# Litianyu141/Gen-FVGN-steady

Measured on AMD Instinct MI355X. Metric: training iters/sec, 50k-cell cylinder mesh (fwd + loss + bwd + Adam, batch resident in HBM), higher is better.
Workload: dtype f32

## Files before the change

### gen-fvgn-steady_amd/csrc/dw.hip

```cpp
#include <stdlib.h>
#include "gfv_common.h"
#include "gfv_prof.h"
#include "gfv_split.h"
#include "../../include/gfv.h"

__device__ int g_gfv_status_flags = 0;

extern "C" int gfv_status_flags(int32_t* flags_out) {
  int v = 0;
  if (hipMemcpyFromSymbol(&v, HIP_SYMBOL(g_gfv_status_flags), sizeof(int)) != hipSuccess) return GFV_ERR_LAUNCH;
  if (v) {
    const int zero = 0;
    if (hipMemcpyToSymbol(HIP_SYMBOL(g_gfv_status_flags), &zero, sizeof(int)) != hipSuccess) return GFV_ERR_LAUNCH;
  }
  if (flags_out) *flags_out = v;
  return GFV_OK;
}

int* gfv_internal_status_ptr() {
  static int* p = nullptr;
  if (!p) {
    void* q = nullptr;
    if (hipGetSymbolAddress(&q, HIP_SYMBOL(g_gfv_status_flags)) == hipSuccess) p = static_cast<int*>(q);
  }
// ... 186 lines not shown
    __syncthreads();
    buf ^= 1;
  }

  float* ws = A.ws + (size_t)slab * A.ws_stride + T.out_off;
#pragma unroll
  for (int i = 0; i < 4; ++i)
#pragma unroll
    for (int j = 0; j < 4; ++j)
#pragma unroll
      for (int reg = 0; reg < 4; ++reg) {
        const int n = 64 * wn + 16 * i + 4 * q + reg;
        const int k = 64 * wk + 16 * j + nl;
        if (FULL || (n < T.n_out && k < T.width)) ws[(size_t)n * T.ld_out + k] = acc[i][j][reg];
      }

  if (T.db_off >= 0) {
    float* red = lds;
    *reinterpret_cast<float4*>(&red[rg * LDT + col]) = dbacc;
    __syncthreads();
    if (tid < T.n_out) {
      float s = 0.f;
#pragma unroll
      for (int r = 0; r < 8; ++r) s += red[r * LDT + tid];
      A.ws[(size_t)slab * A.ws_stride + T.db_off + tid] = s;
    }
  }
}


constexpr int HBLK = 1024;
constexpr int HOP = 16 * HBLK;
constexpr int HBUF = 2 * HOP;
#ifdef GFV_DW_SINGLEBUF
constexpr int HSTAGE = HBUF;
#else
constexpr int HSTAGE = 2 * HBUF;
#endif

template <bool FULL, bool BF>
__device__ __forceinline__ void dw_body_h(const DwLaunch& A, const gfv_dw_tile_t& Tin, unsigned char* lds) {
  gfv_dw_tile_t T = Tin;
  const bool colscale = (T.a_op & GFV_DW_COLSCALE) != 0;
  T.a_op &= 7;
  const int tid = threadIdx.x, wave = tid >> 6, lane = tid & 63, nl = lane & 15, q = lane >> 4;
  const int wn = wave >> 1, wk = wave & 1;
  const int slab = blockIdx.x;
  const int kpad = FULL ? 128 : ((T.width + 15) & ~15);
  const int npad = FULL ? 128 : ((T.n_out + 15) & ~15);
  const bool gvec = FULL || (((T.ldg & 3) == 0) && ((T.n_out & 3) == 0));
  const bool avec = FULL || (((T.ld & 3) == 0) && ((T.width & 3) == 0));
  const int c4 = tid & 31, r4 = tid >> 5;
  const int col = 4 * c4;
  float4 gam = make_float4(1.f, 1.f, 1.f, 1.f), bet = make_float4(0.f, 0.f, 0.f, 0.f);
  if (T.a_op == 2) {
    gam = *reinterpret_cast<const float4*>(T.a_gamma + col);
    bet = *reinterpret_cast<const float4*>(T.a_beta + col);
  }
  const int m_beg = slab * A.rows_per_slab;
  const int m_end = min(m_beg + A.rows_per_slab, A.M);

  float* wred = reinterpret_cast<float*>(lds);
  float sg;
  if (T.gscale) {
    float smin = 8.5070592e37f;
    for (int q = (m_beg >> 4) + tid; q < ((m_end + 15) >> 4); q += 256) smin = fminf(smin, T.gscale[q]);
    smin = gfv_wave_min(smin);
    if (lane == 0) wred[wave] = smin;
    __syncthreads();
    sg = fminf(fminf(wred[0], wred[1]), fminf(wred[2], wred[3]));
    __syncthreads();
  } else {
    float gm = 0.f;
    for (int m = m_beg + r4; m < m_end; m += 64) {
      float4 v[8];
#pragma unroll
      for (int u = 0; u < 8; ++u) v[u] = ld4(T.G, (size_t)min(m + 8 * u, m_end - 1), T.ldg, col, FULL ? 128 : T.n_out, gvec);
#pragma unroll
      for (int u = 0; u < 8; ++u)
        gm = fmaxf(fmaxf(gm, fmaxf(fabsf(v[u].x), fabsf(v[u].y))), fmaxf(fabsf(v[u].z), fabsf(v[u].w)));
    }
    gm = gfv_wave_max(gm);
    if (lane == 0) wred[wave] = gm;
    __syncthreads();
    sg = gfv_pow2_scale(fmaxf(fmaxf(wred[0], wred[1]), fmaxf(wred[2], wred[3])));
    __syncthreads();
  }

  float4 sa = make_float4(1.f, 1.f, 1.f, 1.f);
  if (colscale && m_beg < m_end) {
    float4 cm = make_float4(0.f, 0.f, 0.f, 0.f);
    for (int m = m_beg + r4; m < m_end; m += 64) {
      float4 v[8], b[8];
#pragma unroll
      for (int u = 0; u < 8; ++u) {
        const int mm = min(m + 8 * u, m_end - 1);
        const size_t row = T.idx ? (size_t)T.idx[mm] : (size_t)mm;
        v[u] = ld4(T.A, row, T.ld, col, FULL ? 128 : T.width, avec);
        b[u] = T.in_add ? ld4(T.in_add, row, T.ld, col, FULL ? 128 : T.width, avec) : make_float4(0.f, 0.f, 0.f, 0.f);
      }
#pragma unroll
      for (int u = 0; u < 8; ++u) {
        cm.x = fmaxf(cm.x, fabsf(v[u].x + b[u].x)); cm.y = fmaxf(cm.y, fabsf(v[u].y + b[u].y));
        cm.z = fmaxf(cm.z, fabsf(v[u].z + b[u].z)); cm.w = fmaxf(cm.w, fabsf(v[u].w + b[u].w));
      }
    }
    *reinterpret_cast<float4*>(&wred[r4 * 128 + col]) = cm;
    __syncthreads();
#pragma unroll
    for (int r = 0; r < 8; ++r) {
      const float4 o = *reinterpret_cast<const float4*>(&wred[r * 128 + col]);
      cm.x = fmaxf(cm.x, o.x); cm.y = fmaxf(cm.y, o.y); cm.z = fmaxf(cm.z, o.z); cm.w = fmaxf(cm.w, o.w);
    }
    sa = make_float4(gfv_pow2_scale(cm.x), gfv_pow2_scale(cm.y), gfv_pow2_scale(cm.z), gfv_pow2_scale(cm.w));
    __syncthreads();
  }
  float* inv_sa = reinterpret_cast<float*>(lds + HSTAGE);
  if (r4 == 0) *reinterpret_cast<float4*>(&inv_sa[col]) = make_float4(1.0f / sa.x, 1.0f / sa.y, 1.0f / sa.z, 1.0f / sa.w);
  float amax = 0.f;

  floatx4 acc[4][4];
#pragma unroll
  for (int i = 0; i < 4; ++i)
#pragma unroll
    for (int j = 0; j < 4; ++j) acc[i][j] = floatx4{0.f, 0.f, 0.f, 0.f};
  float4 dbacc = make_float4(0.f, 0.f, 0.f, 0.f);
  float4 greg[4], areg[4], breg[4];
  int nidx[4];
  auto load_idx = [&](int m0) {
#pragma unroll
    for (int p = 0; p < 4; ++p) {
      const int m = min(m0 + 4 * r4 + p, m_end - 1);
      nidx[p] = T.idx ? T.idx[m] : m;
    }
  };
  auto load_sub = [&](int m0) {
    size_t srow[4];
#pragma unroll
    for (int p = 0; p < 4; ++p) srow[p] = (size_t)nidx[p];
#pragma unroll
    for (int p = 0; p < 4; ++p) {
      const int m = min(m0 + 4 * r4 + p, m_end - 1);
      greg[p] = ld4(T.G, (size_t)m, T.ldg, col, FULL ? 128 : T.n_out, gvec);
    }
#pragma unroll
    for (int p = 0; p < 4; ++p) {
      areg[p] = ld4(T.A, srow[p], T.ld, col, FULL ? 128 : T.width, avec);
      if (T.in_add) breg[p] = ld4(T.in_add, srow[p], T.ld, col, FULL ? 128 : T.width, avec);
    }
    load_idx(m0 + SUB);
  };
  const int slot = ((r4 >> 1) * 16) * 16 + 8 * (r4 & 1);
  auto put4 = [&](unsigned char* op, int c, float v0, float v1, float v2, float v3) {
    unsigned h0, h1, l0, l1;
    gfv_split_pair_t<BF>(v0, v1, h0, l0);
    gfv_split_pair_t<BF>(v2, v3, h1, l1);
    unsigned char* b = op + ((c >> 4) * 2) * HBLK + ((c & 15) ^ ((c >> 4) & 3)) * 16 + slot;
    *reinterpret_cast<uint2*>(b) = make_uint2(h0, h1);
    *reinterpret_cast<uint2*>(b + HBLK) = make_uint2(l0, l1);
  };
  auto store_sub = [&](int buf, int m0) {
    unsigned char* Gs = lds + buf * HBUF;
    unsigned char* As = Gs + HOP;
    const float4 zero = make_float4(0.f, 0.f, 0.f, 0.f);
    float4 g[4], a[4];
#pragma unroll
    for (int p = 0; p < 4; ++p) {
      const bool live = (m0 + 4 * r4 + p) < m_end;
      g[p] = greg[p];
      a[p] = areg[p];
      if (T.in_add) { a[p].x += breg[p].x; a[p].y += breg[p].y; a[p].z += breg[p].z; a[p].w += breg[p].w; }
      if (T.a_op == 1) {
        a[p] = make_float4(gfv_gelu(a[p].x), gfv_gelu(a[p].y), gfv_gelu(a[p].z), gfv_gelu(a[p].w));
      } else if (T.a_op == 2) {
        const float mean = gfv_half_sum((a[p].x + a[p].y) + (a[p].z + a[p].w)) * A.ln_inv_n;
        const float dx = a[p].x - mean, dy = a[p].y - mean, dz = a[p].z - mean, dw = a[p].w - mean;
        const float var = (gfv_half_sum((dx * dx + dy * dy) + (dz * dz + dw * dw)) - A.ln_npad * (mean * mean)) * A.ln_inv_n;
        const float rstd = rsqrtf(var + 1e-5f);
        a[p] = make_float4(dx * rstd * gam.x + bet.x, dy * rstd * gam.y + bet.y, dz * rstd * gam.z + bet.z,
                           dw * rstd * gam.w + bet.w);
      }
      if (!live) { g[p] = zero; a[p] = zero; }
      dbacc.x += g[p].x; dbacc.y += g[p].y; dbacc.z += g[p].z; dbacc.w += g[p].w;
      a[p].x *= sa.x; a[p].y *= sa.y; a[p].z *= sa.z; a[p].w *= sa.w;
      amax = fmaxf(fmaxf(amax, fmaxf(fabsf(a[p].x), fabsf(a[p].y))), fmaxf(fabsf(a[p].z), fabsf(a[p].w)));
    }
    put4(Gs, col + 0, g[0].x * sg, g[1].x * sg, g[2].x * sg, g[3].x * sg);
    put4(Gs, col + 1, g[0].y * sg, g[1].y * sg, g[2].y * sg, g[3].y * sg);
    put4(Gs, col + 2, g[0].z * sg, g[1].z * sg, g[2].z * sg, g[3].z * sg);
    put4(Gs, col + 3, g[0].w * sg, g[1].w * sg, g[2].w * sg, g[3].w * sg);
    put4(As, col + 0, a[0].x, a[1].x, a[2].x, a[3].x);
    put4(As, col + 1, a[0].y, a[1].y, a[2].y, a[3].y);
    put4(As, col + 2, a[0].z, a[1].z, a[2].z, a[3].z);
    put4(As, col + 3, a[0].w, a[1].w, a[2].w, a[3].w);
  };

  int buf = 0;
  if (m_beg < m_end) {
    load_idx(m_beg);
    load_sub(m_beg);
    store_sub(0, m_beg);
  }
  __syncthreads();
  for (int m0 = m_beg; m0 < m_end; m0 += SUB) {
    const bool more = m0 + SUB < m_end;
    if (more) load_sub(m0 + SUB);
#ifdef GFV_DW_SINGLEBUF
    const unsigned char* Gs = lds;
#else
    const unsigned char* Gs = lds + buf * HBUF;
#endif
    const unsigned char* As = Gs + HOP;
    gfv_f16x8 gh[4], gl[4], ah[4], al[4];
#pragma unroll
    for (int i = 0; i < 4; ++i) {
      gh[i] = *reinterpret_cast<const gfv_f16x8*>(Gs + ((4 * wn + i) * 2 + 0) * HBLK + (lane ^ i) * 16);
      gl[i] = *reinterpret_cast<const gfv_f16x8*>(Gs + ((4 * wn + i) * 2 + 1) * HBLK + (lane ^ i) * 16);
      ah[i] = *reinterpret_cast<const gfv_f16x8*>(As + ((4 * wk + i) * 2 + 0) * HBLK + (lane ^ i) * 16);
      al[i] = *reinterpret_cast<const gfv_f16x8*>(As + ((4 * wk + i) * 2 + 1) * HBLK + (lane ^ i) * 16);
    }
    if constexpr (BF) {
#pragma unroll
      for (int i = 0; i < 4; ++i)
#pragma unroll
        for (int j = 0; j < 4; ++j)
          if (FULL || (64 * wn + 16 * i < npad && 64 * wk + 16 * j < kpad)) acc[i][j] = gfv_mma_hh<true>(gh[i], ah[j], acc[i][j]);
    } else {
#pragma unroll
      for (int term = 0; term < 3; ++term)
        if (term == 2 || !A.lowp)
#pragma unroll
          for (int i = 0; i < 4; ++i)
#pragma unroll
            for (int j = 0; j < 4; ++j)
              if (FULL || (64 * wn + 16 * i < npad && 64 * wk + 16 * j < kpad))
                acc[i][j] = __builtin_amdgcn_mfma_f32_16x16x32_f16(term == 0 ? gl[i] : gh[i], term == 1 ? al[j] : ah[j],
                                                                   acc[i][j], 0, 0, 0);
    }
#ifdef GFV_DW_SINGLEBUF
    __syncthreads();
    if (more) store_sub(0, m0 + SUB);
    __syncthreads();
#else
    if (more) store_sub(buf ^ 1, m0 + SUB);
    __syncthreads();
    buf ^= 1;
#endif
  }

  if (!(amax <= 65504.f)) atomicOr(&g_gfv_status_flags, GFV_FLAG_DW_RANGE);
  const float inv = 1.0f / sg;
  float* ws = A.ws + (size_t)slab * A.ws_stride + T.out_off;
#pragma unroll
  for (int j = 0; j < 4; ++j) {
    const int k = 64 * wk + 16 * j + nl;
    const float inva = inv_sa[k];
#pragma unroll
    for (int i = 0; i < 4; ++i)
#pragma unroll
      for (int reg = 0; reg < 4; ++reg) {
        const int n = 64 * wn + 16 * i + 4 * q + reg;
        if (FULL || (n < T.n_out && k < T.width)) ws[(size_t)n * T.ld_out + k] = (acc[i][j][reg] * inv) * inva;
      }
  }

  if (T.db_off >= 0) {
    float* red = reinterpret_cast<float*>(lds);
    *reinterpret_cast<float4*>(&red[r4 * LDT + col]) = dbacc;
    __syncthreads();
    if (tid < T.n_out) {
      float s = 0.f;
#pragma unroll
      for (int r = 0; r < 8; ++r) s += red[r * LDT + tid];
      A.ws[(size_t)slab * A.ws_stride + T.db_off + tid] = s;
    }
  }
}

__global__ __launch_bounds__(256, 2) void dw_multi_kernel(const DwLaunch A) {
  __shared__ __attribute__((aligned(16))) float lds[4 * SUB * LDT];
// ... 212 lines not shown
```

### gen-fvgn-steady_amd/csrc/lin1.hip

```cpp
#include <atomic>
#include <cstdlib>

#include "../../include/gfv.h"
#include "gfv_common.h"
#include "gfv_split.h"

int* gfv_internal_status_ptr();
extern "C" int gfv_hidden_size(void);

namespace {

__device__ __forceinline__ float l1_max3_abs(float m, float a, float b) {
  float r;
  asm("v_max3_f32 %0, %1, |%2|, |%3|" : "=v"(r) : "v"(m), "v"(a), "v"(b));
  return r;
}
__device__ __forceinline__ float l1_row_max4(float v) {
  float a, b;
  gfv_lane_xor16(v, a, b);
  v = fmaxf(a, b);
  gfv_lane_xor32(v, a, b);
  return fmaxf(a, b);
}

// ... 327 lines not shown
  }
  __syncthreads();
  float* red = reinterpret_cast<float*>(lds_raw);
#pragma unroll
  for (int nt = 0; nt < 8; ++nt)
#pragma unroll
    for (int r = 0; r < 4; ++r) {
      const float dg = gfv_row16_sum(dgam[nt][r]), db = gfv_row16_sum(dbet[nt][r]);
      if (li == 0) {
        red[(wave * 2 + 0) * 128 + 16 * nt + 4 * g + r] = dg;
        red[(wave * 2 + 1) * 128 + 16 * nt + 4 * g + r] = db;
      }
    }
  __syncthreads();
  {
    const int half = tid >> 8, j = tid & 255;
    const int tile = 2 * blockIdx.x + half;
    if (tile < B.n_tiles && B.ln_partial) {
      const int w0 = 4 * half, which = j >> 7, c = j & 127;
      const float s = (red[((w0 + 0) * 2 + which) * 128 + c] + red[((w0 + 1) * 2 + which) * 128 + c]) +
                      (red[((w0 + 2) * 2 + which) * 128 + c] + red[((w0 + 3) * 2 + which) * 128 + c]);
      B.ln_partial[(size_t)tile * 256 + j] = s;
    }
  }
  (void)status;
}

struct Lin1CsrArgs {
  const float* src[2];
  int src_ld[2];
  const int* rowptr[2];
  const int* col[2];
  float* save[2];
  const void* img;
  const float* wmax;
  float* out;
  int out_ld;
  int M;
};
template <int LOWP>
__global__ __launch_bounds__(512, 2) void lin1_csr_kernel(const Lin1CsrArgs A, int* status) {
  constexpr int KS = 8;
  extern __shared__ __attribute__((aligned(16))) char lds_raw[];
  gfv_uint4* img = reinterpret_cast<gfv_uint4*>(lds_raw);
  const int tid = threadIdx.x, wave = tid >> 6, lane = tid & 63, li = lane & 15, g = lane >> 4;
  {
    const gfv_uint4* src = reinterpret_cast<const gfv_uint4*>(A.img);
    gfv_uint4 t[16];
#pragma unroll
    for (int u = 0; u < 16; ++u) t[u] = src[(size_t)u * 512 + tid];
#pragma unroll
    for (int u = 0; u < 16; ++u) img[u * 512 + tid] = t[u];
  }
  const int nwg = gridDim.x;
  const int wg = (nwg & 7) == 0 ? (int)(blockIdx.x & 7) * (nwg >> 3) + (int)(blockIdx.x >> 3) : (int)blockIdx.x;
  const int m = wg * 128 + 16 * wave + li;
  const bool live = m < A.M;
  const int mc = live ? m : A.M - 1;
  float v[KS][8];
#pragma unroll
  for (int T = 0; T < KS; ++T)
#pragma unroll
    for (int e = 0; e < 8; ++e) v[T][e] = 0.f;
  int kk[2], ee[2], cn0[2], cn1[2];
#pragma unroll
  for (int s = 0; s < 2; ++s) {
// ... 18 lines not shown
      const float* p0 = A.src[s] + (size_t)c0 * (size_t)A.src_ld[s] + 4 * g;
      const float* p1 = A.src[s] + (size_t)c1 * (size_t)A.src_ld[s] + 4 * g;
      if (one[s]) {
#pragma unroll
        for (int t = 0; t < 8; ++t) a0[s][t] = *reinterpret_cast<const float4*>(p0 + 16 * t);
      }
      if (two[s]) {
#pragma unroll
        for (int t = 0; t < 8; ++t) a1[s][t] = *reinterpret_cast<const float4*>(p1 + 16 * t);
      }
    }
#pragma unroll
    for (int s = 0; s < 2; ++s) {
#pragma unroll
      for (int t = 0; t < 8; ++t) {
        float* d = &v[4 * s + (t >> 1)][4 * (t & 1)];
        if (one[s]) { d[0] += a0[s][t].x; d[1] += a0[s][t].y; d[2] += a0[s][t].z; d[3] += a0[s][t].w; }
        if (two[s]) { d[0] += a1[s][t].x; d[1] += a1[s][t].y; d[2] += a1[s][t].z; d[3] += a1[s][t].w; }
      }
      kk[s] = min(kk[s] + 2, ee[s]);
    }
  }
#pragma unroll
  for (int s = 0; s < 2; ++s) {
    if (A.save[s] && live) {
#pragma unroll
      for (int T = 0; T < 4; ++T) {
        float* sp = A.save[s] + (size_t)m * 128 + 32 * T + 4 * g;
        *reinterpret_cast<float4*>(sp) = make_float4(v[4 * s + T][0], v[4 * s + T][1], v[4 * s + T][2], v[4 * s + T][3]);
        *reinterpret_cast<float4*>(sp + 16) = make_float4(v[4 * s + T][4], v[4 * s + T][5], v[4 * s + T][6], v[4 * s + T][7]);
      }
    }
  }
  float m0 = 0.f, m1 = 0.f;
#pragma unroll
  for (int T = 0; T < KS; ++T) {
    m0 = l1_max3_abs(m0, v[T][0], v[T][1]);
    m1 = l1_max3_abs(m1, v[T][2], v[T][3]);
    m0 = l1_max3_abs(m0, v[T][4], v[T][5]);
    m1 = l1_max3_abs(m1, v[T][6], v[T][7]);
  }
  const float sx = gfv_pow2_scale(l1_row_max4(fmaxf(m0, m1)));
  gfv_f16x8 xh[KS], xl[KS];
#pragma unroll
  for (int T = 0; T < KS; ++T) {
    float e[8];
#pragma unroll
    for (int i = 0; i < 8; ++i) e[i] = v[T][i] * sx;
    gfv_uint4 hi, lo;
    gfv_split8_t<LOWP == 2>(e, hi, lo);
    xh[T] = __builtin_bit_cast(gfv_f16x8, hi);
    xl[T] = __builtin_bit_cast(gfv_f16x8, lo);
  }
  const float inv = 1.0f / sx, invw = 1.0f / gfv_pow2_scale(*A.wmax);
  __syncthreads();
#pragma unroll 2
  for (int nt = 0; nt < 8; ++nt) {
    floatx4 acc = {0.f, 0.f, 0.f, 0.f};
#pragma unroll
    for (int T = 0; T < KS; ++T) {
      const gfv_uint4* f = img + (T * 8 + nt) * 128 + lane;
      const gfv_f16x8 wh = __builtin_bit_cast(gfv_f16x8, f[0]);
      if (!LOWP) {
        const gfv_f16x8 wl = __builtin_bit_cast(gfv_f16x8, f[64]);
        acc = __builtin_amdgcn_mfma_f32_16x16x32_f16(wl, xh[T], acc, 0, 0, 0);
        acc = __builtin_amdgcn_mfma_f32_16x16x32_f16(wh, xl[T], acc, 0, 0, 0);
      }
      acc = gfv_mma_hh<LOWP == 2>(wh, xh[T], acc);
    }
    if (live)
      *reinterpret_cast<float4*>(A.out + (size_t)m * A.out_ld + 16 * nt + 4 * g) =
          make_float4((acc[0] * inv) * invw, (acc[1] * inv) * invw, (acc[2] * inv) * invw, (acc[3] * inv) * invw);
  }
  (void)status;
}
// ... 7 lines not shown
static int l1_cus() {
  static int n = 0;
  if (!n) {
    int dev = 0;
    hipDeviceProp_t pr;
    if (hipGetDevice(&dev) == hipSuccess && hipGetDeviceProperties(&pr, dev) == hipSuccess) n = pr.multiProcessorCount;
    if (n <= 0) n = 256;
  }
  return n;
}
static inline bool l1_dyn_lds(const void* fn, int bytes, std::atomic<unsigned long long>& done) {
  int dev = 0;
  if (hipGetDevice(&dev) != hipSuccess) return false;
  const unsigned long long bit = 1ull << (dev & 63);
  if (done.load(std::memory_order_relaxed) & bit) return true;
  if (hipFuncSetAttribute(fn, hipFuncAttributeMaxDynamicSharedMemorySize, bytes) != hipSuccess) return false;
  done.fetch_or(bit);
  return true;
}
}

int gfv_internal_lin1s_try(const gfv_rowtile_args_t* a, int lowp, hipStream_t stream, int dry);
int gfv_internal_lin1_try(const gfv_rowtile_args_t* a, int lowp, hipStream_t stream, int dry) {
  static const int on = l1_env("GFV_LIN1", 1);
  if (on && gfv_internal_lin1s_try(a, lowp, stream, dry)) return 1;
  static const int min_m = l1_env("GFV_LIN1_MIN_M", 1024);
  if (!on || a->nlayers != 1 || a->M < min_m || (a->flags & (GFV_CHAIN_ROW_OWNER | GFV_CHAIN_COLUMN_OWNER))) return 0;
  const gfv_layer_t& L = a->layer[0];
  if (a->nseg == 2 && a->seg[0].csr_rowptr && a->seg[1].csr_rowptr) {
    static const int csr_on = l1_env("GFV_LIN1_CSR", 1);
    if (!csr_on || !L.Wh || !a->wmax || L.op != GFV_OP_NONE || L.save || L.aux || L.bias || L.bias2 || a->in_op != GFV_IN_NONE ||
        a->fin_op != GFV_FIN_PLAIN || L.K != 256 || L.N != 128)
      return 0;
    if (a->in_add || a->in_save || a->gscale || a->fin_presave || a->fin_stats || a->in_stats || a->dw_partial || a->gadd || a->padd ||
        a->in_aux || a->out_nores || a->ln_partial || a->res[0] || a->res[1] || a->res[2])
      return 0;
    if (!a->out[0] || a->out[1] || a->out[2] || (a->out_ld[0] & 3) || !al16(a->out[0])) return 0;
    Lin1CsrArgs B{};
    for (int i = 0; i < 2; ++i) {
      const gfv_seg_t& sg = a->seg[i];
      if (sg.width != 128 || !sg.idx || sg.csr_scale || (sg.ld & 3) || !al16(sg.ptr) || (sg.save && !al16(sg.save))) return 0;
      B.src[i] = sg.ptr; B.src_ld[i] = sg.ld; B.rowptr[i] = sg.csr_rowptr; B.col[i] = sg.idx; B.save[i] = sg.save;
    }
    B.img = L.Wh;
    B.wmax = a->wmax;
    B.out = a->out[0];
    B.out_ld = a->out_ld[0];
    B.M = a->M;
    if (dry) return 1;
    int* st = gfv_internal_status_ptr();
    const dim3 grid((a->M + 127) / 128), blk(512);
#define L1_CSR(LP)                                                                                               \
  do {                                                                                                           \
    static std::atomic<unsigned long long> done{0};                                                              \
    if (!l1_dyn_lds(reinterpret_cast<const void*>(&lin1_csr_kernel<LP>), 131072, done)) return 0;                \
    GFV_LAUNCH((lin1_csr_kernel<LP>), grid, blk, 131072, stream, B, st);                                 \
  } while (0)
    if (lowp == 2) L1_CSR(2);
    else if (lowp) L1_CSR(1);
    else L1_CSR(0);
#undef L1_CSR
    return 1;
  }
  if (a->fin_op == GFV_FIN_LNBWD) {
    static const int lnb_on = l1_env("GFV_LIN1_LNBWD", 1);
    if (!lnb_on || !L.Wh || !a->wmax || L.op != GFV_OP_NONE || L.save || L.aux || L.bias || L.bias2 || a->in_op != GFV_IN_NONE) return 0;
    if (a->nseg != 2 || L.K != 256 || L.N != 128 || a->in_add || a->in_save || a->gscale || a->fin_presave || a->fin_stats || a->in_stats ||
        a->dw_partial || a->gadd || a->padd || a->in_aux || a->out_nores || !a->fin_aux || !a->fin_gamma || !a->ln_partial)
      return 0;
    for (int i = 0; i < 2; ++i) {
      const gfv_seg_t& sg = a->seg[i];
      if (sg.width != 128 || sg.idx || sg.csr_rowptr || sg.csr_scale || sg.save || (sg.ld & 3) || !al16(sg.ptr)) return 0;
    }
    if (!a->out[0] || a->out[1] || a->out[2] || (a->out_ld[0] & 3) || !al16(a->out[0]) || a->res[1] || a->res[2]) return 0;
    if (a->res[0] && ((a->res_ld[0] & 3) || !al16(a->res[0]))) return 0;
// ... 116 lines not shown
```

### gen-fvgn-steady_amd/csrc/lin1s.hip

```cpp
#include <atomic>
#include <cstdlib>

#include "tchain_kernel.h"
#include "gfv_limits.h"

int* gfv_internal_status_ptr();
extern "C" int gfv_hidden_size(void);

namespace {

__device__ __forceinline__ void l1s_barrier() { asm volatile("s_waitcnt lgkmcnt(0)\n\ts_barrier" ::: "memory"); }

struct Lin1sArgs {
  const float* seg[2];
  int seg_ld[2];
  const int* rowptr[2];
  const int* col[2];
  float* save[2];
  const float* in_add;
  float* in_save;
  const void* img;
  const float* wmax;
  const float* bias[2];
  const float* res[2];
  int res_ld[2];
  float* out[2];
  int out_ld[2];
  int M;
  const float* gamma;
  const float* beta;
  float ln_inv_n, ln_npad;
  const float* aux;
  float* gscale;
  float* ln_partial;
};

template <int KS, int TG>
struct L1sLds {
  static constexpr int FRAG = 0;
  static constexpr int SINV = TG * KS * 2048;
  static constexpr int STAT = SINV + TG * 64;
  static constexpr int PART = STAT + TG * 128;
  static constexpr int TOTAL = PART + TG * 16 * 4 * 8;
};

template <int KS, int NP, int IN_OP, int EPI, bool CSR, int LOWP, int TG>
__global__ __launch_bounds__(256, 2) void lin1s_kernel(const Lin1sArgs A, int* status) {
  constexpr int NSEG = KS / 4;
  using LY = L1sLds<KS, TG>;
  constexpr bool BF = LOWP == 2;
  __shared__ __attribute__((aligned(16))) char lds[LY::TOTAL];
  float* sinv = reinterpret_cast<float*>(lds + LY::SINV);
  float* stat = reinterpret_cast<float*>(lds + LY::STAT);
  float* part = reinterpret_cast<float*>(lds + LY::PART);
  const int w = __builtin_amdgcn_readfirstlane(threadIdx.x >> 6);
  const int lane = threadIdx.x & 63, j = lane & 15, g = lane >> 4;
  const int tile = CSR ? gfv_xcd_tile(blockIdx.x, gridDim.x) : (int)blockIdx.x;
  const int row0 = tile * (16 * TG);
  if (row0 >= A.M) return;
  const int ngt = min(TG, (A.M - row0 + 15) >> 4);
  const int c0 = 32 * w + 4 * g;
  const float invw = 1.0f / gfv_pow2_scale(*A.wmax);

  gfv_f16x8 wh[2][KS], wl[2][KS];
  auto load_w = [&](int p) {
    const gfv_f16x8* im = reinterpret_cast<const gfv_f16x8*>(A.img) + (size_t)p * KS * 1024 + (size_t)(2 * w) * 128 + lane;
// ... 104 lines not shown
    if (IN_OP == 1) {
#pragma unroll
      for (int T = 0; T < KS; ++T)
#pragma unroll
        for (int e = 0; e < 8; ++e) v[T][e] = gfv_gelu(v[T][e]);
    }
    if (IN_OP == 2) {
      float sm = 0.f;
#pragma unroll
      for (int T = 0; T < KS; ++T) {
        sm += (v[T][0] + v[T][1]) + (v[T][2] + v[T][3]);
        sm += (v[T][4] + v[T][5]) + (v[T][6] + v[T][7]);
      }
      const float mean = row_sum(sm) * A.ln_inv_n;
      float qq = 0.f;
#pragma unroll
      for (int T = 0; T < KS; ++T) {
        const float d0 = v[T][0] - mean, d1 = v[T][1] - mean, d2 = v[T][2] - mean, d3 = v[T][3] - mean;
        qq += (d0 * d0 + d1 * d1) + (d2 * d2 + d3 * d3);
        const float d4 = v[T][4] - mean, d5 = v[T][5] - mean, d6 = v[T][6] - mean, d7 = v[T][7] - mean;
        qq += (d4 * d4 + d5 * d5) + (d6 * d6 + d7 * d7);
      }
      const float rstd = rsqrtf((row_sum(qq) - A.ln_npad * (mean * mean)) * A.ln_inv_n + 1e-5f);
#pragma unroll
      for (int T = 0; T < KS; ++T) {
        const float4 ga0 = ld4(A.gamma + 32 * T + 4 * g), ga1 = ld4(A.gamma + 32 * T + 16 + 4 * g);
        const float4 be0 = ld4(A.beta + 32 * T + 4 * g), be1 = ld4(A.beta + 32 * T + 16 + 4 * g);
        v[T][0] = (v[T][0] - mean) * rstd * ga0.x + be0.x; v[T][1] = (v[T][1] - mean) * rstd * ga0.y + be0.y;
        v[T][2] = (v[T][2] - mean) * rstd * ga0.z + be0.z; v[T][3] = (v[T][3] - mean) * rstd * ga0.w + be0.w;
        v[T][4] = (v[T][4] - mean) * rstd * ga1.x + be1.x; v[T][5] = (v[T][5] - mean) * rstd * ga1.y + be1.y;
        v[T][6] = (v[T][6] - mean) * rstd * ga1.z + be1.z; v[T][7] = (v[T][7] - mean) * rstd * ga1.w + be1.w;
      }
    }
    float m0 = 0.f, m1 = 0.f;
#pragma unroll
    for (int T = 0; T < KS; ++T) {
      m0 = max3_abs(m0, v[T][0], v[T][1]);
      m1 = max3_abs(m1, v[T][2], v[T][3]);
      m0 = max3_abs(m0, v[T][4], v[T][5]);
      m1 = max3_abs(m1, v[T][6], v[T][7]);
    }
    const float sx = gfv_pow2_scale(row_max4(fmaxf(m0, m1)));
    if (A.gscale) {
      const float sg = gfv_row16_min(sx);
      if (lane == 0) A.gscale[(size_t)(row0 >> 4) + w] = sg;
    }
    if (g == 0) sinv[w * 16 + j] = 1.0f / sx;
    gfv_uint4* dst = reinterpret_cast<gfv_uint4*>(lds + LY::FRAG + (size_t)w * KS * 2048) + lane;
#pragma unroll
    for (int T = 0; T < KS; ++T) {
      float e[8];
#pragma unroll
      for (int i = 0; i < 8; ++i) e[i] = v[T][i] * sx;
      gfv_uint4 hi, lo;
      gfv_split8_t<BF>(e, hi, lo);
      dst[(2 * T) * 64] = hi;
      if (!LOWP) dst[(2 * T + 1) * 64] = lo;
    }
    if (EPI == 2) {
      float y[8][4];
#pragma unroll
      for (int nt = 0; nt < 8; ++nt) {
        const float4 t = ld4(A.aux + mr * 128 + 16 * nt + 4 * g);
        y[nt][0] = t.x; y[nt][1] = t.y; y[nt][2] = t.z; y[nt][3] = t.w;
      }
      float sm = 0.f;
#pragma unroll
      for (int nt = 0; nt < 8; ++nt) sm += (y[nt][0] + y[nt][1]) + (y[nt][2] + y[nt][3]);
      const float mean = row_sum(sm) * A.ln_inv_n;
      float qq = 0.f;
#pragma unroll
      for (int nt = 0; nt < 8; ++nt) {
        const float d0 = y[nt][0] - mean, d1 = y[nt][1] - mean, d2 = y[nt][2] - mean, d3 = y[nt][3] - mean;
        qq += (d0 * d0 + d1 * d1) + (d2 * d2 + d3 * d3);
      }
      const float rstd = rsqrtf((row_sum(qq) - A.ln_npad * (mean * mean)) * A.ln_inv_n + 1e-5f);
// ... 138 lines not shown
  }
  (void)status;
}

inline bool l1s_al16(const void* p) { return (reinterpret_cast<size_t>(p) & 15) == 0; }

}

int gfv_internal_lin1s_try(const gfv_rowtile_args_t* a, int lowp, hipStream_t stream, int dry) {
  const int on = gfv_internal_limit(GFV_LIM_LIN1S_ON);
  const int max_m = gfv_internal_limit(GFV_LIM_LIN1S_MAX_M);
  if (!on || a->nlayers != 1 || a->M > max_m || a->M < 1 || (a->flags & (GFV_CHAIN_ROW_OWNER | GFV_CHAIN_COLUMN_OWNER))) return 0;
  const gfv_layer_t& L = a->layer[0];
  if (!L.Wh || !a->wmax || L.save || L.bias2 && !l1s_al16(L.bias2)) return 0;
  if (a->fin_presave || a->fin_stats || a->in_stats || a->dw_partial || a->gadd || a->padd || a->in_aux || a->out_nores) return 0;
  Lin1sArgs B{};
  B.img = L.Wh;
  B.wmax = a->wmax;
  B.M = a->M;
  {
    const int hs = gfv_hidden_size();
    const int h = (hs > 0 && hs < 128) ? hs : 128;
    B.ln_inv_n = 1.0f / (float)h;
    B.ln_npad = (float)(128 - h);
  }
  int* st = gfv_internal_status_ptr();
  const bool csr = (a->nseg == 2 && a->seg[0].csr_rowptr && a->seg[1].csr_rowptr) || (a->nseg == 1 && a->seg[0].csr_rowptr);
  int epi = 0, iop = 0, ks = 0, np = 0, tg = 2;
  if (csr) {
    const bool one = a->nseg == 1;
    if (L.op != GFV_OP_NONE || L.aux || L.bias || a->in_op != GFV_IN_NONE || a->fin_op != GFV_FIN_PLAIN ||
        L.K != (one ? 128 : 256) || L.N != (one ? 256 : 128))
      return 0;
    if (a->in_add || a->in_save || a->gscale || a->ln_partial || a->res[0] || a->res[1] || a->res[2]) return 0;
    if (!a->out[0] || (one ? !a->out[1] : a->out[1] != nullptr) || a->out[2] || (a->out_ld[0] & 3) || !l1s_al16(a->out[0])) return 0;
    if (one && ((a->out_ld[1] & 3) || !l1s_al16(a->out[1]))) return 0;
    for (int i = 0; i < a->nseg; ++i) {
      const gfv_seg_t& sg = a->seg[i];
      if (sg.width != 128 || !sg.idx || sg.csr_scale || (sg.ld & 3) || !l1s_al16(sg.ptr) || (sg.save && !l1s_al16(sg.save))) return 0;
      B.seg[i] = sg.ptr; B.seg_ld[i] = sg.ld; B.rowptr[i] = sg.csr_rowptr; B.col[i] = sg.idx; B.save[i] = sg.save;
    }
    B.out[0] = a->out[0]; B.out_ld[0] = a->out_ld[0];
    if (one) { B.out[1] = a->out[1]; B.out_ld[1] = a->out_ld[1]; }
    ks = one ? 4 : 8; np = one ? 2 : 1;
  } else {
    if (a->nseg < 1 || a->nseg > 2 || L.K != 128 * a->nseg || (L.N != 128 && L.N != 256) || (a->nseg == 2 && L.N != 128)) return 0;
    for (int i = 0; i < a->nseg; ++i) {
      const gfv_seg_t& s = a->seg[i];
      if (s.width != 128 || s.idx || s.csr_rowptr || s.csr_scale || s.save || (s.ld & 3) || !l1s_al16(s.ptr)) return 0;
      B.seg[i] = s.ptr; B.seg_ld[i] = s.ld;
    }
    if (a->fin_op == GFV_FIN_LNBWD) {
      if (L.op != GFV_OP_NONE || L.aux || L.bias || a->in_op != GFV_IN_NONE || a->nseg != 2 || L.N != 128) return 0;
      if (a->in_add || a->in_save || a->gscale || !a->fin_aux || !a->fin_gamma || !a->ln_partial) return 0;
      if (!l1s_al16(a->fin_aux) || !l1s_al16(a->fin_gamma) || !l1s_al16(a->ln_partial)) return 0;
      B.aux = a->fin_aux; B.gamma = a->fin_gamma; B.ln_partial = a->ln_partial;
      epi = 2; tg = 4;
    } else {
      if (a->fin_op != GFV_FIN_PLAIN || a->ln_partial) return 0;
      const bool dgelu = L.op == GFV_OP_MUL_DGELU;
      if (L.op != GFV_OP_NONE && !dgelu) return 0;
      if (dgelu ? (!L.aux || !l1s_al16(L.aux) || L.bias || L.bias2 || a->in_op != GFV_IN_NONE) : (L.aux != nullptr)) return 0;
      if (a->in_op != GFV_IN_NONE && a->in_op != GFV_IN_GELU && a->in_op != GFV_IN_LN) return 0;
      if (a->in_op == GFV_IN_LN && (a->nseg != 1 || !a->in_gamma || !a->in_beta || !l1s_al16(a->in_gamma) || !l1s_al16(a->in_beta) || a->in_add || a->in_save))
        return 0;
      if (a->gscale && (a->nseg != 1 || (dgelu && L.N == 128 && !a->res[0]))) return 0;
      if (a->in_add && (a->nseg != 1 || !l1s_al16(a->in_add))) return 0;
      if (a->in_save && (a->nseg != 1 || !l1s_al16(a->in_save))) return 0;
      B.in_add = a->in_add; B.in_save = a->in_save; B.gscale = a->gscale;
      B.gamma = a->in_gamma; B.beta = a->in_beta; B.aux = L.aux;
      epi = dgelu ? 1 : 0;
      iop = a->in_op == GFV_IN_GELU ? 1 : (a->in_op == GFV_IN_LN ? 2 : 0);
    }
// ... 43 lines not shown
```

### gen-fvgn-steady_amd/gfv/engine.py

```python
from __future__ import annotations

import contextlib
import os

import torch

from . import cmdlist
from . import lib as L
from . import ops
from .ops import LayerSpec, Seg

_MODE = {"explicit": 0, "implicit": 1, "imex": 2}


def _empty(dev, *shape):
    return torch.empty(shape, dtype=torch.float32, device=dev)


def pick_concurrent_stream(priority=0, candidates=8):
    if torch.cuda.is_current_stream_capturing():
        return torch.cuda.Stream(priority=priority)
    main = torch.cuda.current_stream()
    cycles = 400_000

# ... 588 lines not shown
            return x_out, e_out, None
        return x_out, e_out, dict(sv_e=sv_e, sv_n=sv_n, prefix=prefix)

    def _edge_tmp(self, dev):
        if self._etmp is None or self._etmp[0].flat.device != dev:
            e = GradStore(["W1c", "b1", "W2", "b2", "W3", "b3"], [(128, 128), (128,), (128, 128), (128,), (128, 128), (128,)], dev)
            n = GradStore(["W1ab"], [(128, 256)], dev)
            self._etmp = (e, n)
        return self._etmp

    def edge_bwd_factored(self, P, sv, G, grads, pl, gadd):
        prefix, M, N = sv["prefix"], sv["M"], pl.N
        names = self._mlp_names(prefix, True)
        W1, W2, W3 = P[names[0]], P[names[2]], P[names[4]]
        dev = W1.device
        W3t, W2t, W1ct, Wabt = self._T(W3), self._T(W2), self._T(W1, perm="c"), self._T(W1, perm="ab")
        e = sv["segs"][0].t
        if self.fuse_dw and sv.get("fused", sv.get("stats") is not None) and e.stride(0) == 128 and G.stride(0) == 128:
            fused = self._edge_bwd_fused(P, sv, G, grads, pl, gadd, names, (W3t, W2t, W1ct, Wabt))
            if fused is not None:
                return fused
        self._rematerialize(P, sv)
        gz2, gz1, g3, g_e_in = (_empty(dev, M, 128) for _ in range(4))
        part = _empty(dev, ops.ln_rows(M), 2, 128)
        gs = _empty(dev, 3, ops.gscale_ld(M))
        have = ops.rowtile_chain(M, [Seg(G)],
                                 [LayerSpec(W3t, None, L.OP_MUL_DGELU, save=gz2, aux=sv["z2"]),
                                  LayerSpec(W2t, None, L.OP_MUL_DGELU, save=gz1, aux=sv["z1"]), LayerSpec(W1ct)],
                                 [g_e_in], res=[G], in_op=L.IN_LNBWD, in_gamma=P[names[6]], in_aux=sv["y3"], in_save=g3,
                                 ln_partial=part, gadd=gadd[0], gadd_s=gadd[1], gadd_r=gadd[2], gscale=gs, in_stats=sv.get("stats"))
        tiles_n = ops.last_ln_rows()
        s0, s1, s2 = (gs[0], gs[1], gs[2]) if have else (None, None, None)
        g_nb = _empty(dev, N, 128)
        if self.csr_fuse and (self._fuse_mask & 4):
            G_s, G_r = _empty(dev, N, 128), _empty(dev, N, 128)
            ops.rowtile_chain(N, [Seg(gz1, csr=(pl.s_rowptr, pl.s_col), save=G_s), Seg(gz1, csr=(pl.r_rowptr, pl.r_col), save=G_r)],
                              [LayerSpec(Wabt)], [g_nb])
        else:
            G_s = ops.seg_gather_sum(gz1, pl.s_rowptr, pl.s_col, N)
            G_r = ops.seg_gather_sum(gz1, pl.r_rowptr, pl.r_col, N)
            ops.rowtile_chain(N, [Seg(G_s), Seg(G_r)], [LayerSpec(Wabt)], [g_nb])
        nb = sv["nb"]
        def side():
            tmpE, tmpN = self._edge_tmp(dev)
            gW1 = grads.view(names[0])
            lib = L.load()
            self._workspace(lib.gfv_dw_multi_workspace_floats(M, 3, tmpE.block("W1c", "b3")[1])
                            + lib.gfv_dw_multi_workspace_floats(N, 2, tmpN.block("W1ab", "W1ab")[1]) + 8, dev)
            w1, slabs1, blen1, used = self._dw_block(tmpE, [("W1c", "b1", 1), ("W2", "b2", 1), ("W3", "b3", 1)],
                                                     [self._tile(gz1, 128, Seg(e), gscale=s2),
                                                      self._tile(gz2, 128, Seg(sv["z1"]), a_op=1, gscale=s1),
                                                      self._tile(g3, 128, Seg(sv["z2"]), a_op=1, gscale=s0)], M, reduce=False)
            w2, slabs2, blen2, _ = self._dw_block(tmpN, [("W1ab", None, 2)],
                                                  [self._tile(G_s, 128, Seg(nb)), self._tile(G_r, 128, Seg(nb))], N,
                                                  reduce=False, ws_offset=used)
            assert w2 == w1 + 4 * used
            off, length = grads.block(names[1], names[5])
            o2, l2 = tmpE.block("b1", "b3")
            assert l2 == length
            ops.reduce_multi([
                dict(partial=w1, out=gW1.data_ptr() + 4 * 256, n_chunks=slabs1, chunk_stride=blen1, rows=128, cols=128, ld_out=384),
                dict(partial=w1 + 4 * o2, out=grads.flat.data_ptr() + 4 * off, n_chunks=slabs1, chunk_stride=blen1, rows=1, cols=l2),
                dict(partial=w2, out=gW1.data_ptr(), n_chunks=slabs2, chunk_stride=blen2, rows=128, cols=256, ld_out=384),
                dict(partial=part, out=self._gview2(grads, names[6], names[7]), n_chunks=tiles_n, chunk_stride=256, rows=1,
                     cols=256)])
        self.defer(side, gz1, gz2, g3, G_s, G_r, nb, e, part, gs, sv["z1"], sv["z2"])
        return g_nb, g_e_in

    def _edge_bwd_fused(self, P, sv, G, grads, pl, gadd, names, Wt):
        M, N = sv["M"], pl.N
        W3t, W2t, W1ct, Wabt = Wt
        dev = G.device
        e = sv["segs"][0].t
        lib = L.load()
        nwg = lib.gfv_rowtile_dw_partials_m(M)
        lean = sv["z2"] is None
        FL = L.DW_FUSED_FLOATS
        dwp = _empty(dev, nwg, FL)
        gz1, g_e_in = _empty(dev, M, 128), _empty(dev, M, 128)
        layers = [LayerSpec(W3t, None, L.OP_MUL_DGELU, aux=sv["z2"]), LayerSpec(W2t, None, L.OP_MUL_DGELU, save=gz1, aux=sv["z1"]),
                  LayerSpec(W1ct)]
        gs = _empty(dev, 3, ops.gscale_ld(M))
        kw = dict(res=[G], in_op=L.IN_LNBWD, in_gamma=P[names[6]], in_aux=sv["y3"], in_stats=sv["stats"], gadd=gadd[0], gadd_s=gadd[1],
                  gadd_r=gadd[2], dw_partial=dwp, gscale=gs,
                  rc=(P[names[2]], P[names[3]], P[names[4]], P[names[5]]) if lean else None)
        if not ops.rowtile_chain(M, [Seg(G)], layers, [g_e_in], query_fused=True, **kw):
            return None
        ops.rowtile_chain(M, [Seg(G)], layers, [g_e_in], **kw)
        g_nb = _empty(dev, N, 128)
        if self.csr_fuse and (self._fuse_mask & 4):
            G_s, G_r = _empty(dev, N, 128), _empty(dev, N, 128)
            ops.rowtile_chain(N, [Seg(gz1, csr=(pl.s_rowptr, pl.s_col), save=G_s), Seg(gz1, csr=(pl.r_rowptr, pl.r_col), save=G_r)],
                              [LayerSpec(Wabt)], [g_nb])
        else:
            G_s = ops.seg_gather_sum(gz1, pl.s_rowptr, pl.s_col, N)
            G_r = ops.seg_gather_sum(gz1, pl.r_rowptr, pl.r_col, N)
            ops.rowtile_chain(N, [Seg(G_s), Seg(G_r)], [LayerSpec(Wabt)], [g_nb])
        nb = sv["nb"]

        def side():
            tmpE, tmpN = self._edge_tmp(dev)
            gW1 = grads.view(names[0])
            base = dwp.data_ptr()
            piece = lambda off, out, rows, cols, ld_out=None: dict(partial=base + 4 * off, out=out, n_chunks=nwg, chunk_stride=FL,
                                                                   rows=rows, cols=cols, ld_in=cols, ld_out=cols if ld_out is None else ld_out)
            pieces = [piece(16384 + 128, self._gview2(grads, names[2], names[3]), 1, 16384 + 128),
                      piece(0, self._gview2(grads, names[4], names[5]), 1, 16384 + 128),
                      piece(2 * 16384 + 256, self._gview2(grads, names[6], names[7]), 1, 256)]
            lay = [("W1c", "b1", 1)]
            self._workspace(lib.gfv_dw_multi_workspace_floats(M, 1, tmpE.block("W1c", "b1")[1])
                            + lib.gfv_dw_multi_workspace_floats(N, 2, tmpN.block("W1ab", "W1ab")[1]) + 8, dev)
            w1, slabs1, blen1, used = self._dw_block(tmpE, lay, [self._tile(gz1, 128, Seg(e), gscale=gs[2])], M, reduce=False)
            ob1, lb1 = tmpE.block("b1", "b1")
            pieces += [dict(partial=w1, out=gW1.data_ptr() + 4 * 256, n_chunks=slabs1, chunk_stride=blen1, rows=128, cols=128, ld_out=384),
                       dict(partial=w1 + 4 * ob1, out=grads.view(names[1]), n_chunks=slabs1, chunk_stride=blen1, rows=1, cols=128)]
            w2, slabs2, blen2, _ = self._dw_block(tmpN, [("W1ab", None, 2)],
                                                  [self._tile(G_s, 128, Seg(nb)), self._tile(G_r, 128, Seg(nb))], N, reduce=False,
                                                  ws_offset=used)
            pieces.append(dict(partial=w2, out=gW1.data_ptr(), n_chunks=slabs2, chunk_stride=blen2, rows=128, cols=256, ld_out=384))
            ops.reduce_multi(pieces)
        self.defer(side, dwp, gz1, e, G_s, G_r, nb, gs)
        return g_nb, g_e_in

    def gn_bwd(self, P, sv, g_x_out, g_e_out, grads, pl):
        N, E = pl.N, pl.E
        dev = g_x_out.device
        prefix = sv["prefix"]
        W1n = P[f"{prefix}.nb_module.net.0.0.weight"]
        W1t = self._T(W1n, perm=True)
        g_x_in, g_nbm = _empty(dev, N, 128), _empty(dev, N, 64)
        self.mlp3_bwd(P, sv["sv_n"], g_x_out, grads, outs=[g_x_in, (g_nbm, 64)], res=[g_x_out, None], W1t=W1t)
        g_agg = ops.seg_gather_sum(g_nbm, pl.n_rowptr, pl.n_col_node, N, src_scale=pl.inv_deg)
        if "nb" in sv["sv_e"]:
            g_nb, g_e_in = self.edge_bwd_factored(P, sv["sv_e"], g_e_out, grads, pl, (g_agg, pl.es, pl.er))
        else:
            gnb2, g_e_in = _empty(dev, E, 256), _empty(dev, E, 128)
            self.mlp3_bwd(P, sv["sv_e"], g_e_out, grads, outs=[(gnb2, 256), (gnb2.data_ptr() + 512, 256), g_e_in],
                          res=[None, None, g_e_out], gadd=(g_agg, pl.es, pl.er))
            g_nb = ops.seg_gather_sum(gnb2.view(2 * E, 128), pl.n_rowptr, pl.n_col_edge2, N)
        ops.seg_gather_sum(g_nb, pl.n_rowptr, pl.n_col_node, N, out=g_x_in, accumulate=True)
        last = self._defer_mode and getattr(self, "_last_gn", False)
        tail_main, tail_split = self._tail_cfg(pl)
        self.flush(on_main=last and tail_main >= 3, split=tail_split if last else 0)
        return g_x_in, g_e_in

    def trans_fwd(self, P, prefix, xg, emb, pl, keep=True):
        lib = L.load()
        st = L.stream_ptr()
        N, B = pl.N, pl.B
        dev = xg.device
        a = f"{prefix}.Attn"
        fx_in, fx_mid, x_mid = _empty(dev, N, 128), _empty(dev, N, 128), _empty(dev, N, 128)
        ops.rowtile_chain(N, [Seg(xg)],
                          [LayerSpec(P[f"{a}.in_project_fx.weight"], P[f"{a}.in_project_fx.bias"],
# ... 520 lines not shown
```

Measured before the change: 286.2.

## Emit per-segment gradient scales from CSR rowtile and prefetch dW tiles earlier

The CSR-fused rowtile kernels (lin1, lin1s) now compute per-16-row power-of-two scales for each gathered segment and write them to a gscale buffer. The dW kernel can then read these instead of rescanning G_s/G_r for their max. The dW kernel also issues the first sub-tile's global loads before the scale reduction so that latency overlaps the reduction. It replaces __syncthreads with an lgkmcnt-only wait plus barrier and drops the single-buffer compile path. The cost is extra stores in the rowtile kernels and a new path-flag dependency in the engine.

Result: no change. 287.8, median of 6 (+0.6%).

```diff
diff --git a/gen-fvgn-steady_amd/csrc/dw.hip b/gen-fvgn-steady_amd/csrc/dw.hip
--- a/gen-fvgn-steady_amd/csrc/dw.hip
+++ b/gen-fvgn-steady_amd/csrc/dw.hip
@@ -242,11 +242,9 @@
 constexpr int HBLK = 1024;
 constexpr int HOP = 16 * HBLK;
 constexpr int HBUF = 2 * HOP;
-#ifdef GFV_DW_SINGLEBUF
-constexpr int HSTAGE = HBUF;
-#else
 constexpr int HSTAGE = 2 * HBUF;
-#endif
+
+__device__ __forceinline__ void dw_lds_barrier() { asm volatile("s_waitcnt lgkmcnt(0)\n\ts_barrier" ::: "memory"); }
 
 template <bool FULL, bool BF>
 __device__ __forceinline__ void dw_body_h(const DwLaunch& A, const gfv_dw_tile_t& Tin, unsigned char* lds) {
@@ -270,16 +268,46 @@
   const int m_beg = slab * A.rows_per_slab;
   const int m_end = min(m_beg + A.rows_per_slab, A.M);
 
+  float4 greg[4], areg[4], breg[4];
+  int nidx[4];
+  auto load_idx = [&](int m0) {
+#pragma unroll
+    for (int p = 0; p < 4; ++p) {
+      const int m = min(m0 + 4 * r4 + p, m_end - 1);
+      nidx[p] = T.idx ? T.idx[m] : m;
+    }
+  };
+  auto load_sub = [&](int m0) {
+    size_t srow[4];
+#pragma unroll
+    for (int p = 0; p < 4; ++p) srow[p] = (size_t)nidx[p];
+#pragma unroll
+    for (int p = 0; p < 4; ++p) {
+      const int m = min(m0 + 4 * r4 + p, m_end - 1);
+      greg[p] = ld4(T.G, (size_t)m, T.ldg, col, FULL ? 128 : T.n_out, gvec);
+    }
+#pragma unroll
+    for (int p = 0; p < 4; ++p) {
+      areg[p] = ld4(T.A, srow[p], T.ld, col, FULL ? 128 : T.width, avec);
+      if (T.in_add) breg[p] = ld4(T.in_add, srow[p], T.ld, col, FULL ? 128 : T.width, avec);
+    }
+    load_idx(m0 + SUB);
+  };
   float* wred = reinterpret_cast<float*>(lds);
   float sg;
   if (T.gscale) {
-    float smin = 8.5070592e37f;
-    for (int q = (m_beg >> 4) + tid; q < ((m_end + 15) >> 4); q += 256) smin = fminf(smin, T.gscale[q]);
+    const int q0 = (m_beg >> 4) + tid, q1 = (m_end + 15) >> 4;
+    float smin = q0 < q1 ? T.gscale[q0] : 8.5070592e37f;
+    if (m_beg < m_end) {
+      load_idx(m_beg);
+      load_sub(m_beg);
+    }
+    for (int q = q0 + 256; q < q1; q += 256) smin = fminf(smin, T.gscale[q]);
     smin = gfv_wave_min(smin);
     if (lane == 0) wred[wave] = smin;
-    __syncthreads();
+    dw_lds_barrier();
     sg = fminf(fminf(wred[0], wred[1]), fminf(wred[2], wred[3]));
-    __syncthreads();
+    dw_lds_barrier();
   } else {
     float gm = 0.f;
     for (int m = m_beg + r4; m < m_end; m += 64) {
@@ -290,11 +318,15 @@
       for (int u = 0; u < 8; ++u)
         gm = fmaxf(fmaxf(gm, fmaxf(fabsf(v[u].x), fabsf(v[u].y))), fmaxf(fabsf(v[u].z), fabsf(v[u].w)));
     }
+    if (m_beg < m_end) {
+      load_idx(m_beg);
+      load_sub(m_beg);
+    }
     gm = gfv_wave_max(gm);
     if (lane == 0) wred[wave] = gm;
-    __syncthreads();
+    dw_lds_barrier();
     sg = gfv_pow2_scale(fmaxf(fmaxf(wred[0], wred[1]), fmaxf(wred[2], wred[3])));
-    __syncthreads();
+    dw_lds_barrier();
   }
 
   float4 sa = make_float4(1.f, 1.f, 1.f, 1.f);
@@ -335,31 +367,6 @@
 #pragma unroll
     for (int j = 0; j < 4; ++j) acc[i][j] = floatx4{0.f, 0.f, 0.f, 0.f};
   float4 dbacc = make_float4(0.f, 0.f, 0.f, 0.f);
-  float4 greg[4], areg[4], breg[4];
-  int nidx[4];
-  auto load_idx = [&](int m0) {
-#pragma unroll
-    for (int p = 0; p < 4; ++p) {
-      const int m = min(m0 + 4 * r4 + p, m_end - 1);
-      nidx[p] = T.idx ? T.idx[m] : m;
-    }
-  };
-  auto load_sub = [&](int m0) {
-    size_t srow[4];
-#pragma unroll
-    for (int p = 0; p < 4; ++p) srow[p] = (size_t)nidx[p];
-#pragma unroll
-    for (int p = 0; p < 4; ++p) {
-      const int m = min(m0 + 4 * r4 + p, m_end - 1);
-      greg[p] = ld4(T.G, (size_t)m, T.ldg, col, FULL ? 128 : T.n_out, gvec);
-    }
-#pragma unroll
-    for (int p = 0; p < 4; ++p) {
-      areg[p] = ld4(T.A, srow[p], T.ld, col, FULL ? 128 : T.width, avec);
-      if (T.in_add) breg[p] = ld4(T.in_add, srow[p], T.ld, col, FULL ? 128 : T.width, avec);
-    }
-    load_idx(m0 + SUB);
-  };
   const int slot = ((r4 >> 1) * 16) * 16 + 8 * (r4 & 1);
   auto put4 = [&](unsigned char* op, int c, float v0, float v1, float v2, float v3) {
     unsigned h0, h1, l0, l1;
@@ -406,20 +413,12 @@
   };
 
   int buf = 0;
-  if (m_beg < m_end) {
-    load_idx(m_beg);
-    load_sub(m_beg);
-    store_sub(0, m_beg);
-  }
+  if (m_beg < m_end) store_sub(0, m_beg);
   __syncthreads();
   for (int m0 = m_beg; m0 < m_end; m0 += SUB) {
     const bool more = m0 + SUB < m_end;
     if (more) load_sub(m0 + SUB);
-#ifdef GFV_DW_SINGLEBUF
-    const unsigned char* Gs = lds;
-#else
     const unsigned char* Gs = lds + buf * HBUF;
-#endif
     const unsigned char* As = Gs + HOP;
     gfv_f16x8 gh[4], gl[4], ah[4], al[4];
 #pragma unroll
@@ -447,15 +446,9 @@
                 acc[i][j] = __builtin_amdgcn_mfma_f32_16x16x32_f16(term == 0 ? gl[i] : gh[i], term == 1 ? al[j] : ah[j],
                                                                    acc[i][j], 0, 0, 0);
     }
-#ifdef GFV_DW_SINGLEBUF
-    __syncthreads();
-    if (more) store_sub(0, m0 + SUB);
-    __syncthreads();
-#else
     if (more) store_sub(buf ^ 1, m0 + SUB);
     __syncthreads();
     buf ^= 1;
-#endif
   }
 
   if (!(amax <= 65504.f)) atomicOr(&g_gfv_status_flags, GFV_FLAG_DW_RANGE);
diff --git a/gen-fvgn-steady_amd/csrc/lin1.hip b/gen-fvgn-steady_amd/csrc/lin1.hip
--- a/gen-fvgn-steady_amd/csrc/lin1.hip
+++ b/gen-fvgn-steady_amd/csrc/lin1.hip
@@ -383,6 +383,7 @@
   const int* rowptr[2];
   const int* col[2];
   float* save[2];
+  float* gscale[2];
   const void* img;
   const float* wmax;
   float* out;
@@ -467,15 +468,24 @@
       }
     }
   }
-  float m0 = 0.f, m1 = 0.f;
-#pragma unroll
-  for (int T = 0; T < KS; ++T) {
-    m0 = l1_max3_abs(m0, v[T][0], v[T][1]);
-    m1 = l1_max3_abs(m1, v[T][2], v[T][3]);
-    m0 = l1_max3_abs(m0, v[T][4], v[T][5]);
-    m1 = l1_max3_abs(m1, v[T][6], v[T][7]);
-  }
-  const float sx = gfv_pow2_scale(l1_row_max4(fmaxf(m0, m1)));
+  float sm[2];
+#pragma unroll
+  for (int s = 0; s < 2; ++s) {
+    float m0 = 0.f, m1 = 0.f;
+#pragma unroll
+    for (int T = 4 * s; T < 4 * s + 4; ++T) {
+      m0 = l1_max3_abs(m0, v[T][0], v[T][1]);
+      m1 = l1_max3_abs(m1, v[T][2], v[T][3]);
+      m0 = l1_max3_abs(m0, v[T][4], v[T][5]);
+      m1 = l1_max3_abs(m1, v[T][6], v[T][7]);
+    }
+    sm[s] = l1_row_max4(fmaxf(m0, m1));
+    if (A.gscale[s]) {
+      const float sg = gfv_row16_min(gfv_pow2_scale(sm[s]));
+      if (lane == 0 && 16 * (wg * 8 + wave) < A.M) A.gscale[s][wg * 8 + wave] = sg;
+    }
+  }
+  const float sx = gfv_pow2_scale(fmaxf(sm[0], sm[1]));
   gfv_f16x8 xh[KS], xl[KS];
 #pragma unroll
   for (int T = 0; T < KS; ++T) {
@@ -549,7 +559,7 @@
     if (!csr_on || !L.Wh || !a->wmax || L.op != GFV_OP_NONE || L.save || L.aux || L.bias || L.bias2 || a->in_op != GFV_IN_NONE ||
         a->fin_op != GFV_FIN_PLAIN || L.K != 256 || L.N != 128)
       return 0;
-    if (a->in_add || a->in_save || a->gscale || a->fin_presave || a->fin_stats || a->in_stats || a->dw_partial || a->gadd || a->padd ||
+    if (a->in_add || a->in_save || a->fin_presave || a->fin_stats || a->in_stats || a->dw_partial || a->gadd || a->padd ||
         a->in_aux || a->out_nores || a->ln_partial || a->res[0] || a->res[1] || a->res[2])
       return 0;
     if (!a->out[0] || a->out[1] || a->out[2] || (a->out_ld[0] & 3) || !al16(a->out[0])) return 0;
@@ -558,6 +568,7 @@
       const gfv_seg_t& sg = a->seg[i];
       if (sg.width != 128 || !sg.idx || sg.csr_scale || (sg.ld & 3) || !al16(sg.ptr) || (sg.save && !al16(sg.save))) return 0;
       B.src[i] = sg.ptr; B.src_ld[i] = sg.ld; B.rowptr[i] = sg.csr_rowptr; B.col[i] = sg.idx; B.save[i] = sg.save;
+      B.gscale[i] = (a->gscale && sg.save) ? a->gscale + (size_t)i * a->gscale_ld : nullptr;
     }
     B.img = L.Wh;
     B.wmax = a->wmax;
diff --git a/gen-fvgn-steady_amd/csrc/lin1s.hip b/gen-fvgn-steady_amd/csrc/lin1s.hip
--- a/gen-fvgn-steady_amd/csrc/lin1s.hip
+++ b/gen-fvgn-steady_amd/csrc/lin1s.hip
@@ -32,6 +32,7 @@
   float ln_inv_n, ln_npad;
   const float* aux;
   float* gscale;
+  float* seg_gscale[2];
   float* ln_partial;
 };
 
@@ -202,16 +203,23 @@
         v[T][6] = (v[T][6] - mean) * rstd * ga1.z + be1.z; v[T][7] = (v[T][7] - mean) * rstd * ga1.w + be1.w;
       }
     }
-    float m0 = 0.f, m1 = 0.f;
+    float mh[2] = {0.f, 0.f};
 #pragma unroll
     for (int T = 0; T < KS; ++T) {
-      m0 = max3_abs(m0, v[T][0], v[T][1]);
-      m1 = max3_abs(m1, v[T][2], v[T][3]);
+      float m0 = max3_abs(0.f, v[T][0], v[T][1]), m1 = max3_abs(0.f, v[T][2], v[T][3]);
       m0 = max3_abs(m0, v[T][4], v[T][5]);
       m1 = max3_abs(m1, v[T][6], v[T][7]);
-    }
-    const float sx = gfv_pow2_scale(row_max4(fmaxf(m0, m1)));
-    if (A.gscale) {
+      mh[T >> 2] = fmaxf(mh[T >> 2], fmaxf(m0, m1));
+    }
+    const float sx = gfv_pow2_scale(row_max4(fmaxf(mh[0], mh[1])));
+    if (CSR && NSEG == 2) {
+#pragma unroll
+      for (int s = 0; s < 2; ++s)
+        if (A.seg_gscale[s]) {
+          const float sg = gfv_row16_min(gfv_pow2_scale(row_max4(mh[s])));
+          if (lane == 0) A.seg_gscale[s][(size_t)(row0 >> 4) + w] = sg;
+        }
+    } else if (A.gscale) {
       const float sg = gfv_row16_min(sx);
       if (lane == 0) A.gscale[(size_t)(row0 >> 4) + w] = sg;
     }
@@ -416,13 +424,14 @@
     if (L.op != GFV_OP_NONE || L.aux || L.bias || a->in_op != GFV_IN_NONE || a->fin_op != GFV_FIN_PLAIN ||
         L.K != (one ? 128 : 256) || L.N != (one ? 256 : 128))
       return 0;
-    if (a->in_add || a->in_save || a->gscale || a->ln_partial || a->res[0] || a->res[1] || a->res[2]) return 0;
+    if (a->in_add || a->in_save || (a->gscale && one) || a->ln_partial || a->res[0] || a->res[1] || a->res[2]) return 0;
     if (!a->out[0] || (one ? !a->out[1] : a->out[1] != nullptr) || a->out[2] || (a->out_ld[0] & 3) || !l1s_al16(a->out[0])) return 0;
     if (one && ((a->out_ld[1] & 3) || !l1s_al16(a->out[1]))) return 0;
     for (int i = 0; i < a->nseg; ++i) {
       const gfv_seg_t& sg = a->seg[i];
       if (sg.width != 128 || !sg.idx || sg.csr_scale || (sg.ld & 3) || !l1s_al16(sg.ptr) || (sg.save && !l1s_al16(sg.save))) return 0;
       B.seg[i] = sg.ptr; B.seg_ld[i] = sg.ld; B.rowptr[i] = sg.csr_rowptr; B.col[i] = sg.idx; B.save[i] = sg.save;
+      B.seg_gscale[i] = (a->gscale && !one && sg.save) ? a->gscale + (size_t)i * a->gscale_ld : nullptr;
     }
     B.out[0] = a->out[0]; B.out_ld[0] = a->out_ld[0];
     if (one) { B.out[1] = a->out[1]; B.out_ld[1] = a->out_ld[1]; }
diff --git a/gen-fvgn-steady_amd/gfv/engine.py b/gen-fvgn-steady_amd/gfv/engine.py
--- a/gen-fvgn-steady_amd/gfv/engine.py
+++ b/gen-fvgn-steady_amd/gfv/engine.py
@@ -644,10 +644,14 @@
         tiles_n = ops.last_ln_rows()
         s0, s1, s2 = (gs[0], gs[1], gs[2]) if have else (None, None, None)
         g_nb = _empty(dev, N, 128)
+        gs_n = None
         if self.csr_fuse and (self._fuse_mask & 4):
             G_s, G_r = _empty(dev, N, 128), _empty(dev, N, 128)
+            gs_n = _empty(dev, 3, ops.gscale_ld(N))
             ops.rowtile_chain(N, [Seg(gz1, csr=(pl.s_rowptr, pl.s_col), save=G_s), Seg(gz1, csr=(pl.r_rowptr, pl.r_col), save=G_r)],
-                              [LayerSpec(Wabt)], [g_nb])
+                              [LayerSpec(Wabt)], [g_nb], gscale=gs_n)
+            if not (L.load().gfv_rowtile_last_path() & 32):
+                gs_n = None
         else:
             G_s = ops.seg_gather_sum(gz1, pl.s_rowptr, pl.s_col, N)
             G_r = ops.seg_gather_sum(gz1, pl.r_rowptr, pl.r_col, N)
@@ -664,7 +668,8 @@
                                                       self._tile(gz2, 128, Seg(sv["z1"]), a_op=1, gscale=s1),
                                                       self._tile(g3, 128, Seg(sv["z2"]), a_op=1, gscale=s0)], M, reduce=False)
             w2, slabs2, blen2, _ = self._dw_block(tmpN, [("W1ab", None, 2)],
-                                                  [self._tile(G_s, 128, Seg(nb)), self._tile(G_r, 128, Seg(nb))], N,
+                                                  [self._tile(G_s, 128, Seg(nb), gscale=None if gs_n is None else gs_n[0]),
+                                                   self._tile(G_r, 128, Seg(nb), gscale=None if gs_n is None else gs_n[1])], N,
                                                   reduce=False, ws_offset=used)
             assert w2 == w1 + 4 * used
             off, length = grads.block(names[1], names[5])
@@ -676,7 +681,7 @@
                 dict(partial=w2, out=gW1.data_ptr(), n_chunks=slabs2, chunk_stride=blen2, rows=128, cols=256, ld_out=384),
                 dict(partial=part, out=self._gview2(grads, names[6], names[7]), n_chunks=tiles_n, chunk_stride=256, rows=1,
                      cols=256)])
-        self.defer(side, gz1, gz2, g3, G_s, G_r, nb, e, part, gs, sv["z1"], sv["z2"])
+        self.defer(side, gz1, gz2, g3, G_s, G_r, nb, e, part, gs, gs_n, sv["z1"], sv["z2"])
         return g_nb, g_e_in
 
     def _edge_bwd_fused(self, P, sv, G, grads, pl, gadd, names, Wt):
@@ -700,10 +705,14 @@
             return None
         ops.rowtile_chain(M, [Seg(G)], layers, [g_e_in], **kw)
         g_nb = _empty(dev, N, 128)
+        gs_n = None
         if self.csr_fuse and (self._fuse_mask & 4):
             G_s, G_r = _empty(dev, N, 128), _empty(dev, N, 128)
+            gs_n = _empty(dev, 3, ops.gscale_ld(N))
             ops.rowtile_chain(N, [Seg(gz1, csr=(pl.s_rowptr, pl.s_col), save=G_s), Seg(gz1, csr=(pl.r_rowptr, pl.r_col), save=G_r)],
-                              [LayerSpec(Wabt)], [g_nb])
+                              [LayerSpec(Wabt)], [g_nb], gscale=gs_n)
+            if not (L.load().gfv_rowtile_last_path() & 32):
+                gs_n = None
         else:
             G_s = ops.seg_gather_sum(gz1, pl.s_rowptr, pl.s_col, N)
             G_r = ops.seg_gather_sum(gz1, pl.r_rowptr, pl.r_col, N)
@@ -727,11 +736,12 @@
             pieces += [dict(partial=w1, out=gW1.data_ptr() + 4 * 256, n_chunks=slabs1, chunk_stride=blen1, rows=128, cols=128, ld_out=384),
                        dict(partial=w1 + 4 * ob1, out=grads.view(names[1]), n_chunks=slabs1, chunk_stride=blen1, rows=1, cols=128)]
             w2, slabs2, blen2, _ = self._dw_block(tmpN, [("W1ab", None, 2)],
-                                                  [self._tile(G_s, 128, Seg(nb)), self._tile(G_r, 128, Seg(nb))], N, reduce=False,
-                                                  ws_offset=used)
+                                                  [self._tile(G_s, 128, Seg(nb), gscale=None if gs_n is None else gs_n[0]),
+                                                   self._tile(G_r, 128, Seg(nb), gscale=None if gs_n is None else gs_n[1])], N,
+                                                  reduce=False, ws_offset=used)
             pieces.append(dict(partial=w2, out=gW1.data_ptr(), n_chunks=slabs2, chunk_stride=blen2, rows=128, cols=256, ld_out=384))
             ops.reduce_multi(pieces)
-        self.defer(side, dwp, gz1, e, G_s, G_r, nb, gs)
+        self.defer(side, dwp, gz1, e, G_s, G_r, nb, gs, gs_n)
         return g_nb, g_e_in
 
     def gn_bwd(self, P, sv, g_x_out, g_e_out, grads, pl):
```
